# google-research/multinerf

Measured on NVIDIA H100. Metric: train-step rays/sec @16384 rays x (64+64+32) samples, higher is better.
Workload: dtype bf16

## Files before the change

### include/mnrf.h

```cpp
#ifndef MNRF_H_
#define MNRF_H_

#include <stddef.h>
#include <stdint.h>

#ifdef __cplusplus
extern "C" {
#endif

typedef uint16_t mnrf_bf16;
typedef void* mnrf_stream;

#define MNRF_ABI_VERSION 2

int mnrf_abi_version(void);
const char* mnrf_last_error(void);
int mnrf_device_ok(void);
int mnrf_num_sms(void);

typedef struct {
  int32_t num_rays, num_prev, num_samples;
  int32_t use_dilation;
  float dilation, domain_lo, domain_hi;
  float anneal, resample_padding;
// ... 33 lines not shown
                     mnrf_stream stream);

enum { MNRF_GEMM_FWD = 0, MNRF_GEMM_DGRAD = 1, MNRF_GEMM_WGRAD = 2 };
enum { MNRF_ACT_NONE = 0, MNRF_ACT_RELU = 1, MNRF_ACT_SOFTPLUS = 2, MNRF_ACT_SILU = 3 };

typedef struct {
  int32_t mode, act;
  int64_t m;
  int32_t n, k;
  int64_t lda, ldb, ldc, ldmask;
  int64_t ldmaskbits;
  int64_t ldadd;
  int64_t mask_mod;
  int32_t impl;
} mnrf_gemm_desc;

int mnrf_gemm(const mnrf_gemm_desc* d, const mnrf_bf16* a, const mnrf_bf16* b, const float* bias,
              const float* rowv, const float* colv, const mnrf_bf16* mask, uint32_t* maskbits,
              float* colsum, const mnrf_bf16* addend, mnrf_bf16* z, int64_t ldz, void* out, mnrf_stream stream);

int mnrf_gemm_wgrad(const mnrf_gemm_desc* d, const mnrf_bf16* a, const mnrf_bf16* b, float* bsum,
                    const float* side_w, float* side_aw, float* out, mnrf_stream stream);

typedef struct {
  int32_t block_n;
  int32_t staged;
  int32_t mask_tma;
  int32_t smooth;
  int32_t side;
  int32_t splits;
  int32_t tiles;
  int32_t grid;
  int32_t pingpong;
} mnrf_gemm_instance;
int mnrf_gemm_plan(const mnrf_gemm_desc* d, const mnrf_bf16* a, const mnrf_bf16* b, const float* bias,
                   const float* rowv, const float* colv, const mnrf_bf16* mask, const uint32_t* maskbits,
                   const float* colsum, const mnrf_bf16* addend, const mnrf_bf16* z, int64_t ldz, const void* out,
                   const float* bsum, const float* side_w, const float* side_aw, mnrf_gemm_instance* plan);

#define MNRF_CHAIN_MAX_LAYERS 8
enum { MNRF_CHAIN_FWD = 0, MNRF_CHAIN_BWD = 1 };

typedef struct {
  const mnrf_bf16* w;
  int64_t ldw;
  const float* bias;
  uint32_t* maskbits;
  int64_t ldmaskbits;
  float* colsum;
  mnrf_bf16* out;
  int64_t ldo;
  int32_t n_stream, stream_col0, stream_kb0;
  int32_t n_res, res_kb0;
  int32_t reserved;
} mnrf_chain_layer;

typedef struct {
  int32_t mode, num_layers;
  int32_t width;
  int32_t stream_cols;
  int64_t m;
  const mnrf_bf16* stream;
  int64_t ldstream;
  const float* head_w;
  const float* head_b;
  float* head_out;
// ... 200 lines not shown
```

### multinerf_b200/csrc/gemm_tc.cu

```cuda
#include <cuda.h>

#include <stdlib.h>
#include <string.h>

#include <algorithm>

#include "tc_common.cuh"

namespace mnrf {

constexpr int BLOCK_M = 128;
constexpr int BLOCK_K = 64;
constexpr int A_STAGE_BYTES = BLOCK_M * BLOCK_K * 2;
constexpr int NUM_THREADS = 384;
constexpr int CS_MAX = 1024;
constexpr int gemm_stages(int bn) { return bn == 256 ? 4 : bn == 128 ? 6 : 8; }
constexpr int STAGING_BLOCK_BYTES = 64 * 128;
constexpr int staging_blocks(int mode, int bn, bool ts) {
  return !ts ? 0 : (mode == MNRF_GEMM_FWD && bn >= 128) ? 2 : 1;
}
constexpr int mask_words(int bn) { return bn >= 128 ? bn / 32 : 0; }
constexpr int MASK_BUFS = 2;
constexpr int dgrad_smem_bytes(int bn) { return 8 * bn * 4 + MASK_BUFS * BLOCK_M * mask_words(bn) * 4; }
constexpr int SIDE_SCRATCH = 96 * 8;
// ... 75 lines not shown
          w = r < 32 ? wl : wh;
        }
        if (r < BLOCK_K) {
          const uint4 v = ld_shared_v4((base + r * 128) ^ ((r & 7) << 4));
          const uint32_t u[4] = {v.x, v.y, v.z, v.w};
#pragma unroll
          for (int q = 0; q < 4; ++q) {
            acc[2 * q] = fmaf(w, bf16_lo(u[q]), acc[2 * q]);
            acc[2 * q + 1] = fmaf(w, bf16_hi(u[q]), acc[2 * q + 1]);
          }
        }
      }
      __syncwarp();
      if (lane == 0) mbar_arrive(&empty_bar[slot % STAGES]);
    }
    if (own < BLOCK_K && kb0 < kb1) {
      if (NT > 32) named_bar_sync(4, NT); else __syncwarp();
#pragma unroll
      for (int e = 0; e < 8; ++e) st_shared_u32(scratch + (t * 8 + e) * 4, __float_as_uint(acc[e]));
      if (NT > 32) named_bar_sync(4, NT); else __syncwarp();
      const int64_t col0 = WEIGHTED ? (int64_t)m_blk * BLOCK_M : (int64_t)n_blk * COLS;
      float* out = WEIGHTED ? p.side_aw : p.bsum;
      for (int col = t; col < COLS; col += NT) {
        if (WEIGHTED && col0 + col >= p.m) break;
        float sum = 0.f;
#pragma unroll
        for (int g = 0; g < G; ++g) sum += __uint_as_float(ld_shared_u32(scratch + (g * COLS + col) * 4));
        atomicAdd(out + col0 + col, sum);
      }
    }
  }
}

template <int MODE, int NC, bool TS, int SB, bool SMOOTH>
__device__ __forceinline__ void gemm_epilogue(const GemmParams& p, const CUtensorMap* tmap_c, const float (&acc)[NC / 2],
                                              int m_blk, int r0, int ncol0, int wg, uint8_t* smem_c, bool mask_tma,
                                              uint32_t m_tile, bool do_cs, uint32_t cs_lane) {
  constexpr int MW = mask_words(NC);
  const int lane = threadIdx.x & 31;
  const int r_in = r0 + (16 * ((threadIdx.x >> 5) & 3) + (lane >> 2));
  const int cq = 2 * (lane & 3);
  const bool leader = (threadIdx.x & 127) == 0;
  const uint32_t c_row = smem_u32(smem_c) + wg * (SB * STAGING_BLOCK_BYTES) + (r_in - r0) * 128 + (cq << 1);
  const uint32_t m_row = m_tile + r_in * (MW * 4);
  int64_t rows[2];
  bool row_ok[2];
  float rv[2] = {0.f, 0.f};
  const uint32_t* mrow[2] = {nullptr, nullptr};
#pragma unroll
  for (int h = 0; h < 2; ++h) {
    rows[h] = (int64_t)m_blk * BLOCK_M + r_in + 8 * h;
    row_ok[h] = rows[h] < p.m;
    if (MODE == MNRF_GEMM_DGRAD && row_ok[h]) {
      if (p.rowv) rv[h] = p.rowv[rows[h]];
      if (p.maskbits && !mask_tma)
        mrow[h] = p.maskbits + (p.mask_mod > 0 ? rows[h] % p.mask_mod : rows[h]) * p.ldmaskbits;
    }
  }
  uint32_t bits[2] = {0u, 0u};
  uint32_t mw[2] = {0u, 0u};
#pragma unroll
  for (int i = 0; i < NC / 8; ++i) {
    const int col = ncol0 + 8 * i + cq;
    if (TS && SB == 1 && (i & 7) == 0) {
      if (leader) tma_store_wait_read<0>();
      named_bar_sync(2 + wg, 128);
    }
    if (MODE == MNRF_GEMM_DGRAD && p.maskbits && (i & 3) == 0) {
#pragma unroll
      for (int h = 0; h < 2; ++h)
        mw[h] = mask_tma ? ld_shared_u32(m_row + (8 * h * MW + (i >> 2)) * 4)
                         : row_ok[h] ? __ldg(mrow[h] + (col >> 5)) : 0u;
    }
    float v[2][2];
#pragma unroll
    for (int h = 0; h < 2; ++h) { v[h][0] = acc[4 * i + 2 * h]; v[h][1] = acc[4 * i + 2 * h + 1]; }
    if (MODE == MNRF_GEMM_FWD) {
      if (p.bias) {
        const float2 b = __ldg(reinterpret_cast<const float2*>(p.bias + col));
#pragma unroll
        for (int h = 0; h < 2; ++h) { v[h][0] += b.x; v[h][1] += b.y; }
      }
      if constexpr (SMOOTH) {
#pragma unroll
        for (int h = 0; h < 2; ++h) {
          if (p.mask && row_ok[h])
            *reinterpret_cast<uint32_t*>(const_cast<__nv_bfloat16*>(p.mask) + rows[h] * p.ldmask + col) =
                pack_bf16(v[h][0], v[h][1]);
          v[h][0] = act_fwd(p.act, v[h][0]);
          v[h][1] = act_fwd(p.act, v[h][1]);
        }
      } else if (p.act == MNRF_ACT_RELU) {
#pragma unroll
        for (int h = 0; h < 2; ++h)
#pragma unroll
          for (int e = 0; e < 2; ++e) {
            v[h][e] = relu_nan(v[h][e]);
            bits[h] |= (v[h][e] > 0.f ? 1u : 0u) << ((8 * i + cq + e) & 31);
          }
      }
    } else {
      float2 cv = make_float2(0.f, 0.f);
      if (p.rowv) cv = __ldg(reinterpret_cast<const float2*>(p.colv + col));
#pragma unroll
      for (int h = 0; h < 2; ++h) {
        if (p.rowv) { v[h][0] += rv[h] * cv.x; v[h][1] += rv[h] * cv.y; }
        if constexpr (SMOOTH) {
          if (row_ok[h]) {
            const int64_t zr = p.mask_mod > 0 ? rows[h] % p.mask_mod : rows[h];
            const uint32_t zz = __ldg(reinterpret_cast<const unsigned int*>(p.mask + zr * p.ldmask + col));
            v[h][0] *= act_d1(p.act, bf16_lo(zz));
            v[h][1] *= act_d1(p.act, bf16_hi(zz));
          }
        } else if (p.maskbits) {
          if (!((mw[h] >> (col & 31)) & 1u)) v[h][0] = 0.f;
          if (!((mw[h] >> ((col + 1) & 31)) & 1u)) v[h][1] = 0.f;
        } else if (p.mask && row_ok[h]) {
          const uint32_t mm = __ldg(reinterpret_cast<const unsigned int*>(p.mask + rows[h] * p.ldmask + col));
          if (!(bf16_lo(mm) > 0.f)) v[h][0] = 0.f;
          if (!(bf16_hi(mm) > 0.f)) v[h][1] = 0.f;
        }
        if (p.addend && row_ok[h]) {
          const uint32_t aa = __ldg(reinterpret_cast<const unsigned int*>(p.addend + rows[h] * p.ldadd + col));
          v[h][0] += bf16_lo(aa);
          v[h][1] += bf16_hi(aa);
        }
      }
      if (do_cs) {
        const bool hi = (lane >> 2) & 1;
        const float s0 = v[0][0] + v[1][0], s1 = v[0][1] + v[1][1];
        float t = (hi ? s1 : s0) + __shfl_xor_sync(0xffffffffu, hi ? s0 : s1, 4);
        t += __shfl_xor_sync(0xffffffffu, t, 8);
        t += __shfl_xor_sync(0xffffffffu, t, 16);
        if (lane < 8) {
          const uint32_t a = cs_lane + 8 * i * 4;
          st_shared_u32(a, __float_as_uint(__uint_as_float(ld_shared_u32(a)) + t));
        }
      }
    }
#pragma unroll
    for (int h = 0; h < 2; ++h) {
      if (TS) {
        st_shared_u32(c_row + ((i >> 3) & (SB - 1)) * STAGING_BLOCK_BYTES + h * (8 * 128) +
                          (((i & 7) ^ ((lane >> 2) & 7)) << 4),
                      pack_bf16(v[h][0], v[h][1]));
      } else if (row_ok[h]) {
        *reinterpret_cast<uint32_t*>(reinterpret_cast<__nv_bfloat16*>(p.out) + rows[h] * p.ldc + col) =
            pack_bf16(v[h][0], v[h][1]);
      }
    }
    if (MODE == MNRF_GEMM_FWD && p.act == MNRF_ACT_RELU && p.maskbits && (i & 3) == 3) {
#pragma unroll
      for (int h = 0; h < 2; ++h) {
        bits[h] |= __shfl_xor_sync(0xffffffffu, bits[h], 1);
        bits[h] |= __shfl_xor_sync(0xffffffffu, bits[h], 2);
        if ((lane & 3) == ((i >> 2) & 3) && row_ok[h]) p.maskbits[rows[h] * p.ldmaskbits + (col >> 5)] = bits[h];
        bits[h] = 0u;
      }
    }
    if (TS && (i & 7) == 7) {
      fence_proxy_async();
      if (SB == 2 && leader) tma_store_wait_read<0>();
      named_bar_sync(2 + wg, 128);
      if (leader) {
        tma_store_2d(tmap_c, smem_c + (wg * SB + ((i >> 3) & (SB - 1))) * STAGING_BLOCK_BYTES, ncol0 + 8 * (i & ~7),
                     (int)((int64_t)m_blk * BLOCK_M + r0));
        tma_store_commit();
      }
    }
  }
}

template <int MODE, int BN, bool TS, bool SIDE, bool SMOOTH = false>
__global__ void __launch_bounds__(NUM_THREADS, 1)
gemm_tc_kernel(const __grid_constant__ CUtensorMap tmap_a, const __grid_constant__ CUtensorMap tmap_b,
               const __grid_constant__ CUtensorMap tmap_c, const __grid_constant__ CUtensorMap tmap_m,
               const GemmParams p) {
  constexpr int STAGES = gemm_stages(BN);
  constexpr int B_STAGE = BN * BLOCK_K * 2;
  constexpr bool kWgrad = (MODE == MNRF_GEMM_WGRAD);
  constexpr bool kDgrad = (MODE == MNRF_GEMM_DGRAD);
  constexpr int NACC = BN / 2;
  constexpr int SB = staging_blocks(MODE, BN, TS);
  constexpr int MW = mask_words(BN);
  static_assert(SB < 2 || (BN / 64) % 2 == 0, "block j of every tile must use staging block j % SB");
  static_assert(!SIDE || kWgrad, "side sums are a WGRAD feature");
  static_assert(!SMOOTH || (TS && !kWgrad), "smooth activations are FWD / DGRAD epilogues of the staged store");
  extern __shared__ uint8_t smem_dyn[];
  uint8_t* smem = reinterpret_cast<uint8_t*>((reinterpret_cast<uintptr_t>(smem_dyn) + 1023) & ~uintptr_t(1023));
  uint8_t* smem_a = smem;
  uint8_t* smem_b = smem + STAGES * A_STAGE_BYTES;
  uint8_t* smem_c = smem_b + STAGES * B_STAGE;
  float* cs_s = reinterpret_cast<float*>(smem_c + 2 * SB * STAGING_BLOCK_BYTES);
  float* side_s = cs_s;
  uint32_t* mask_s = reinterpret_cast<uint32_t*>(cs_s + (kDgrad ? 8 * BN : SIDE ? SIDE_SCRATCH : 0));
  uint64_t* full_bar = reinterpret_cast<uint64_t*>(mask_s + (kDgrad ? MASK_BUFS * BLOCK_M * MW : 0));
  uint64_t* empty_bar = full_bar + STAGES;
  uint64_t* mask_full = empty_bar + STAGES;
  uint64_t* mask_empty = mask_full + MASK_BUFS;

  const int warp = threadIdx.x >> 5;
// ... 93 lines not shown
          uint64_t adesc, bdesc;
          if (!kWgrad) {
            adesc = make_smem_desc(sa + c * (64 * 128) + k * (WGMMA_K * 2), 0, 1024);
            bdesc = make_smem_desc(sb + k * (WGMMA_K * 2), 0, 1024);
          } else {
            adesc = make_smem_desc(sa + c * (BLOCK_K * 128) + k * (WGMMA_K * 128), BLOCK_K * 128, 1024);
            bdesc = make_smem_desc(sb + k * (WGMMA_K * 128), BLOCK_K * 128, 1024);
          }
          Wgmma<BN, kWgrad ? 1 : 0, kWgrad ? 1 : 0>::mma(acc, adesc, bdesc, (kb > kb0 || k > 0) ? 1u : 0u);
        }
        wgmma_commit();
        wgmma_wait<1>();
        if (prev >= 0 && lane == 0) mbar_arrive(&empty_bar[prev]);
        prev = (int)stage;
        if (++stage == STAGES) { stage = 0; phase ^= 1; }
      }
      wgmma_wait<0>();
      fence_acc(acc);
      if (prev >= 0 && lane == 0) mbar_arrive(&empty_bar[prev]);

      const int ncol0 = n_blk * BN;
      if (MODE == MNRF_GEMM_WGRAD) {
#pragma unroll
        for (int h = 0; h < 2; ++h) {
          const int64_t row = (int64_t)m_blk * BLOCK_M + r_in + 8 * h;
          if (row >= p.m) continue;
          float* dst = reinterpret_cast<float*>(p.out) + row * p.ldc + ncol0 + cq;
#pragma unroll
          for (int i = 0; i < BN / 8; ++i) atomicAdd(reinterpret_cast<float2*>(dst + 8 * i), make_float2(acc[4 * i + 2 * h], acc[4 * i + 2 * h + 1]));
        }
        continue;
      }
      if (mask_tma) mbar_wait(&mask_full[it % MASK_BUFS], (it / MASK_BUFS) & 1, 5);
      gemm_epilogue<MODE, BN, TS, SB, SMOOTH>(p, &tmap_c, acc, m_blk, 64 * c, ncol0, c, smem_c, mask_tma,
                                              smem_u32(mask_s) + (it % MASK_BUFS) * (BLOCK_M * MW * 4), do_cs, cs_lane);
      if (mask_tma) {
        __syncwarp();
        if (lane == 0) mbar_arrive(&mask_empty[it % MASK_BUFS]);
      }
      const int next = tile + (int)gridDim.x;
      if (do_cs && (next >= total_tiles || next % p.num_n_blocks != n_blk)) {
        named_bar_sync(1, 2 * 128);
        for (int j = threadIdx.x - 128; j < BN; j += 2 * 128) {
          float s = 0.f;
#pragma unroll
          for (int sw = 0; sw < 8; ++sw) {
            s += cs_s[sw * BN + j];
            cs_s[sw * BN + j] = 0.f;
          }
          atomicAdd(p.colsum + ncol0 + j, s);
        }
        named_bar_sync(1, 2 * 128);
      }
    }
    if (TS && (threadIdx.x & 127) == 0) tma_store_wait_all();
  }
}

constexpr int PP_BN = 128;
constexpr int PP_STAGES = 5;
constexpr int PP_SB = 2;
constexpr int PP_MASK_BUFS = 4;
constexpr int pp_smem_bytes(int mode) {
  return PP_STAGES * (A_STAGE_BYTES + PP_BN * BLOCK_K * 2) + 2 * PP_SB * STAGING_BLOCK_BYTES +
         (mode == MNRF_GEMM_DGRAD ? PP_MASK_BUFS * BLOCK_M * mask_words(PP_BN) * 4 : 0) + 256  +
         1024 ;
}

template <int MODE, int BN>
__global__ void __launch_bounds__(NUM_THREADS, 1)
gemm_tc_pingpong_kernel(const __grid_constant__ CUtensorMap tmap_a, const __grid_constant__ CUtensorMap tmap_b,
                        const __grid_constant__ CUtensorMap tmap_c, const __grid_constant__ CUtensorMap tmap_m,
                        const GemmParams p) {
  constexpr int STAGES = PP_STAGES;
  constexpr int B_STAGE = PP_BN * BLOCK_K * 2;
  constexpr int SUB = BN / PP_BN;
  constexpr int MW = mask_words(PP_BN);
  constexpr int SB = PP_SB;
  constexpr bool kDgrad = (MODE == MNRF_GEMM_DGRAD);
  static_assert(MODE != MNRF_GEMM_WGRAD && (BN == 128 || BN == 256), "FWD / DGRAD tiles of 128 or 256 columns");
  extern __shared__ uint8_t smem_dyn[];
  uint8_t* smem = reinterpret_cast<uint8_t*>((reinterpret_cast<uintptr_t>(smem_dyn) + 1023) & ~uintptr_t(1023));
  uint8_t* smem_a = smem;
  uint8_t* smem_b = smem + STAGES * A_STAGE_BYTES;
  uint8_t* smem_c = smem_b + STAGES * B_STAGE;
  uint32_t* mask_s = reinterpret_cast<uint32_t*>(smem_c + 2 * SB * STAGING_BLOCK_BYTES);
  uint64_t* full_bar = reinterpret_cast<uint64_t*>(mask_s + (kDgrad ? PP_MASK_BUFS * BLOCK_M * MW : 0));
  uint64_t* empty_bar = full_bar + STAGES;
  uint64_t* mask_full = empty_bar + STAGES;
  uint64_t* mask_empty = mask_full + PP_MASK_BUFS;
  uint64_t* mma_turn = mask_empty + PP_MASK_BUFS;

  const int lane = threadIdx.x & 31;
  const int wg = threadIdx.x >> 7;
  const int total_tiles = p.num_m_blocks * p.num_n_blocks;
  const int nk = p.num_k_blocks;
  const bool mask_tma = kDgrad && p.mask_tma;

  if (threadIdx.x == 0) {
    prefetch_tmap(&tmap_a);
    prefetch_tmap(&tmap_b);
    prefetch_tmap(&tmap_c);
    if (mask_tma) prefetch_tmap(&tmap_m);
    for (int i = 0; i < STAGES; ++i) {
      mbar_init(&full_bar[i], 1);
      mbar_init(&empty_bar[i], 4);
    }
    for (int i = 0; i < PP_MASK_BUFS; ++i) {
      mbar_init(&mask_full[i], 1);
      mbar_init(&mask_empty[i], 4);
    }
    for (int i = 0; i < 2; ++i) mbar_init(&mma_turn[i], 4);
    fence_barrier_init();
  }
  __syncthreads();
  pdl_launch_dependents();
  pdl_wait();

  if (wg == 0) {
    setmaxnreg_dec<40>();
    if (threadIdx.x == 0) {
      uint32_t stage = 0, phase = 0;
      int it = 0;
      for (int tile = blockIdx.x; tile < total_tiles; tile += gridDim.x) {
        const int n_blk = tile % p.num_n_blocks;
        const int m_blk = tile / p.num_n_blocks;
        for (int s = 0; s < SUB; ++s, ++it) {
          const int ncol0 = n_blk * BN + s * PP_BN;
          if (mask_tma) {
            const int mb = it % PP_MASK_BUFS;
            mbar_wait(&mask_empty[mb], ((it / PP_MASK_BUFS) & 1) ^ 1, 4);
            mbar_expect_tx(&mask_full[mb], BLOCK_M * MW * 4);
            const int64_t r0 = (int64_t)m_blk * BLOCK_M;
            tma_load_2d(mask_s + mb * (BLOCK_M * MW), &tmap_m, &mask_full[mb], ncol0 / 32,
                        (int)(p.mask_mod > 0 ? r0 % p.mask_mod : r0));
          }
          for (int kb = 0; kb < nk; ++kb) {
            mbar_wait(&empty_bar[stage], phase ^ 1, 1);
            mbar_expect_tx(&full_bar[stage], A_STAGE_BYTES + B_STAGE);
            tma_load_2d(smem_a + stage * A_STAGE_BYTES, &tmap_a, &full_bar[stage], kb * BLOCK_K, m_blk * BLOCK_M);
            tma_load_2d(smem_b + stage * B_STAGE, &tmap_b, &full_bar[stage], kb * BLOCK_K, ncol0);
            if (++stage == STAGES) { stage = 0; phase ^= 1; }
          }
        }
      }
    }
  } else {
    setmaxnreg_inc<232>();
    const int c = wg - 1;
    float acc[2][64];
    for (int it = c; ; it += 2) {
      const int tile = blockIdx.x + (it / SUB) * (int)gridDim.x;
      if (tile >= total_tiles) break;
      const int s = it % SUB;
      const int n_blk = tile % p.num_n_blocks;
      const int m_blk = tile / p.num_n_blocks;
      const int ncol0 = n_blk * BN + s * PP_BN;
      const uint32_t slot = (uint32_t)it * (uint32_t)nk;
      uint32_t stage = slot % STAGES, phase = (slot / STAGES) & 1;
      if (it > 0) mbar_wait(&mma_turn[c], ((it - 1) >> 1) & 1, 7);
      int prev = -1;
      fence_acc(acc[0]);
      fence_acc(acc[1]);
      for (int kb = 0; kb < nk; ++kb) {
        mbar_wait(&full_bar[stage], phase, 3);
        const uint32_t sa = smem_u32(smem_a + stage * A_STAGE_BYTES);
        const uint32_t sb = smem_u32(smem_b + stage * B_STAGE);
        wgmma_fence();
#pragma unroll
        for (int k = 0; k < BLOCK_K / WGMMA_K; ++k) {
          const uint64_t bdesc = make_smem_desc(sb + k * (WGMMA_K * 2), 0, 1024);
#pragma unroll
          for (int g = 0; g < 2; ++g)
            Wgmma<PP_BN, 0, 0>::mma(acc[g], make_smem_desc(sa + g * (64 * 128) + k * (WGMMA_K * 2), 0, 1024), bdesc,
                                    (kb > 0 || k > 0) ? 1u : 0u);
        }
        wgmma_commit();
        wgmma_wait<1>();
        if (prev >= 0 && lane == 0) mbar_arrive(&empty_bar[prev]);
        prev = (int)stage;
        if (++stage == STAGES) { stage = 0; phase ^= 1; }
      }
      if (blockIdx.x + ((it + 1) / SUB) * (int)gridDim.x < total_tiles) {
        __syncwarp();
        if (lane == 0) mbar_arrive(&mma_turn[c ^ 1]);
      }
      wgmma_wait<0>();
      fence_acc(acc[0]);
      fence_acc(acc[1]);
      if (prev >= 0 && lane == 0) mbar_arrive(&empty_bar[prev]);

      const uint32_t m_base = smem_u32(mask_s) + (it % PP_MASK_BUFS) * (BLOCK_M * MW * 4);
      if (mask_tma) mbar_wait(&mask_full[it % PP_MASK_BUFS], (it / PP_MASK_BUFS) & 1, 5);
#pragma unroll 1
      for (int g = 0; g < 2; ++g) {
        gemm_epilogue<MODE, PP_BN, true, SB, false>(p, &tmap_c, acc[0], m_blk, 64 * g, ncol0, c, smem_c, mask_tma, m_base,
                                                    false, 0);
#pragma unroll
        for (int e = 0; e < 64; ++e) acc[0][e] = acc[1][e];
      }
      if (mask_tma) {
        __syncwarp();
        if (lane == 0) mbar_arrive(&mask_empty[it % PP_MASK_BUFS]);
      }
    }
    if ((threadIdx.x & 127) == 0) tma_store_wait_all();
  }
}

template <int MODE, int BN>
static int launch_gemm_tc_pingpong(int grid, const CUtensorMap& ta, const CUtensorMap& tb, const CUtensorMap& tc,
                                   const CUtensorMap& tm, const GemmParams& p, cudaStream_t stream) {
  constexpr int kSmem = pp_smem_bytes(MODE);
  static_assert(kSmem <= 232448, "shared memory budget");
  return launch_tc<gemm_tc_pingpong_kernel<MODE, BN>>(grid, NUM_THREADS, kSmem, stream, ta, tb, tc, tm, p);
}

template <int MODE, int BN, bool TS, bool SIDE, bool SMOOTH = false>
static int launch_gemm_tc(int grid, const CUtensorMap& ta, const CUtensorMap& tb, const CUtensorMap& tc,
                          const CUtensorMap& tm, const GemmParams& p, cudaStream_t stream) {
  constexpr int kSmem = smem_bytes(MODE, BN, TS, SIDE);
  static_assert(kSmem <= 232448, "shared memory budget");
  return launch_tc<gemm_tc_kernel<MODE, BN, TS, SIDE, SMOOTH>>(grid, NUM_THREADS, kSmem, stream, ta, tb, tc, tm, p);
}

int gemm_tc_smooth_launch(int mode, int block_n, int grid, const CUtensorMap& ta, const CUtensorMap& tb,
                          const CUtensorMap& tc, const GemmParams& p, cudaStream_t stream);

#ifndef MNRF_GEMM_TC_SMOOTH_UNIT
static int pick_block_n(int n) {
  const int cands[] = {256, 128, 64, 32, 16};
  for (int c : cands)
    if (n % c == 0) return c;
  return 0;
}

static int gemm_tc_plan(const mnrf_gemm_desc* d, const mnrf_bf16* a, const mnrf_bf16* b, const float* bias,
                        const float* colv, const mnrf_bf16* mask, const uint32_t* maskbits, const float* colsum,
                        const mnrf_bf16* addend, const void* out, const float* bsum, const float* side_w,
                        const float* side_aw, const mnrf_bf16* z, int64_t ldz, mnrf_gemm_instance* plan,
                        GemmParams* p) {
  MNRF_CHECK(d->mode == MNRF_GEMM_WGRAD || d->k % BLOCK_K == 0,
             "mnrf_gemm(tc): reduction length %d must be a multiple of %d", d->k, BLOCK_K);
  MNRF_CHECK(d->lda % 8 == 0 && d->ldb % 8 == 0 && ((uintptr_t)a % 16) == 0 && ((uintptr_t)b % 16) == 0,
             "mnrf_gemm(tc): operands must be 16-byte aligned with ld %% 8 == 0");
  const int block_n = pick_block_n(d->n);
  MNRF_CHECK(block_n > 0, "mnrf_gemm(tc): N=%d must be a multiple of 16", d->n);
  if (d->mode == MNRF_GEMM_WGRAD)
// ... 18 lines not shown
  }
  if (bias) MNRF_CHECK(((uintptr_t)bias % 8) == 0, "mnrf_gemm(tc): bias must be 8-byte aligned");
  if (colv) MNRF_CHECK(((uintptr_t)colv % 8) == 0, "mnrf_gemm(tc): colv must be 8-byte aligned");
  const int workers = mnrf_num_sms();
  const int num_m_blocks = (int)((d->m + BLOCK_M - 1) / BLOCK_M);
  const int num_n_blocks = d->n / block_n;
  const int num_k_blocks = (d->k + BLOCK_K - 1) / BLOCK_K;
  int num_splits = 1;
  if (d->mode == MNRF_GEMM_WGRAD) {
    const int out_tiles = num_m_blocks * num_n_blocks;
    const int max_splits = std::min(std::max(1, (2 * workers) / out_tiles), num_k_blocks);
    int splits = max_splits;
    for (int sp = 1; sp <= max_splits; ++sp) {
      const int items = out_tiles * sp;
      const int rounds = (items + workers - 1) / workers;
      if (items * 100 >= rounds * workers * 95) { splits = sp; break; }
    }
    num_splits = splits;
  }
  const int kblocks_per_split = (num_k_blocks + num_splits - 1) / num_splits;
  num_splits = (num_k_blocks + kblocks_per_split - 1) / kblocks_per_split;
  if (d->mode != MNRF_GEMM_WGRAD) {
    MNRF_CHECK(d->ldc % 2 == 0 && ((uintptr_t)out % 4) == 0, "mnrf_gemm(tc): bf16 output must be 4-byte aligned");
    if (mask) MNRF_CHECK(d->ldmask % 2 == 0 && ((uintptr_t)mask % 4) == 0, "mnrf_gemm(tc): mask must be 4-byte aligned");
  } else {
    MNRF_CHECK(d->ldc % 2 == 0 && ((uintptr_t)out % 8) == 0, "mnrf_gemm(tc): fp32 output must be 8-byte aligned");
  }
  const bool ts = d->mode != MNRF_GEMM_WGRAD && block_n >= 64 && ((uintptr_t)out % 16) == 0 && d->ldc % 8 == 0;
  MNRF_CHECK(!smooth || ts, "mnrf_gemm(tc): a smooth activation needs N %% 64 == 0 and a 16-byte aligned output "
             "with a row pitch that is a multiple of 8");
  const bool mask_tma = d->mode == MNRF_GEMM_DGRAD && maskbits && mask_words(block_n) > 0 && d->ldmaskbits % 4 == 0 &&
                        ((uintptr_t)maskbits % 16) == 0 && (d->mask_mod == 0 || d->mask_mod % BLOCK_M == 0);
  const bool pingpong = d->mode != MNRF_GEMM_WGRAD && ts && d->n % PP_BN == 0 && !smooth && !colsum;
  const int tiles = num_m_blocks * num_n_blocks * num_splits;
  plan->block_n = block_n;
  plan->staged = ts;
  plan->mask_tma = mask_tma;
  plan->smooth = smooth;
  plan->side = side;
  plan->splits = num_splits;
  plan->tiles = tiles;
  plan->grid = std::min(tiles, workers);
  plan->pingpong = pingpong;
  p->num_m_blocks = num_m_blocks;
  p->num_n_blocks = num_n_blocks;
  p->num_k_blocks = num_k_blocks;
  p->num_splits = num_splits;
  p->kblocks_per_split = kblocks_per_split;
  return 0;
}

template <int MODE>
static int launch_register_store(int block_n, int grid, const CUtensorMap& ta, const CUtensorMap& tb,
                                 const CUtensorMap& tc, const CUtensorMap& tm, const GemmParams& p,
                                 cudaStream_t stream) {
  switch (block_n) {
    case 256: return launch_gemm_tc<MODE, 256, false, false>(grid, ta, tb, tc, tm, p, stream);
    case 128: return launch_gemm_tc<MODE, 128, false, false>(grid, ta, tb, tc, tm, p, stream);
    case 64: return launch_gemm_tc<MODE, 64, false, false>(grid, ta, tb, tc, tm, p, stream);
    case 32: return launch_gemm_tc<MODE, 32, false, false>(grid, ta, tb, tc, tm, p, stream);
    case 16: return launch_gemm_tc<MODE, 16, false, false>(grid, ta, tb, tc, tm, p, stream);
  }
  set_error("mnrf_gemm(tc): no register-store instance at BN=%d", block_n);
  return 1;
}

static int launch_gemm_tc_plan(int mode, const mnrf_gemm_instance& plan, const CUtensorMap& ta, const CUtensorMap& tb,
                               const CUtensorMap& tc, const CUtensorMap& tm, const GemmParams& p,
                               cudaStream_t stream) {
  const int bn = plan.block_n, grid = plan.grid;
  const bool fwd = mode == MNRF_GEMM_FWD;
  if (plan.pingpong) {
    if (bn == 256)
      return fwd ? launch_gemm_tc_pingpong<MNRF_GEMM_FWD, 256>(grid, ta, tb, tc, tm, p, stream)
                 : launch_gemm_tc_pingpong<MNRF_GEMM_DGRAD, 256>(grid, ta, tb, tc, tm, p, stream);
    if (bn == 128)
      return fwd ? launch_gemm_tc_pingpong<MNRF_GEMM_FWD, 128>(grid, ta, tb, tc, tm, p, stream)
                 : launch_gemm_tc_pingpong<MNRF_GEMM_DGRAD, 128>(grid, ta, tb, tc, tm, p, stream);
  } else if (plan.smooth) {
    return gemm_tc_smooth_launch(mode, bn, grid, ta, tb, tc, p, stream);
  } else if (mode == MNRF_GEMM_WGRAD) {
    if (bn == 256)
      return plan.side ? launch_gemm_tc<MNRF_GEMM_WGRAD, 256, false, true>(grid, ta, tb, tc, tm, p, stream)
                       : launch_gemm_tc<MNRF_GEMM_WGRAD, 256, false, false>(grid, ta, tb, tc, tm, p, stream);
    if (bn == 128)
      return plan.side ? launch_gemm_tc<MNRF_GEMM_WGRAD, 128, false, true>(grid, ta, tb, tc, tm, p, stream)
                       : launch_gemm_tc<MNRF_GEMM_WGRAD, 128, false, false>(grid, ta, tb, tc, tm, p, stream);
    if (bn == 64)
      return plan.side ? launch_gemm_tc<MNRF_GEMM_WGRAD, 64, false, true>(grid, ta, tb, tc, tm, p, stream)
                       : launch_gemm_tc<MNRF_GEMM_WGRAD, 64, false, false>(grid, ta, tb, tc, tm, p, stream);
  } else if (!plan.staged) {
    return fwd ? launch_register_store<MNRF_GEMM_FWD>(bn, grid, ta, tb, tc, tm, p, stream)
               : launch_register_store<MNRF_GEMM_DGRAD>(bn, grid, ta, tb, tc, tm, p, stream);
  } else if (bn == 64) {
    return fwd ? launch_gemm_tc<MNRF_GEMM_FWD, 64, true, false>(grid, ta, tb, tc, tm, p, stream)
               : launch_gemm_tc<MNRF_GEMM_DGRAD, 64, true, false>(grid, ta, tb, tc, tm, p, stream);
  } else if (!fwd) {
    if (bn == 256) return launch_gemm_tc<MNRF_GEMM_DGRAD, 256, true, false>(grid, ta, tb, tc, tm, p, stream);
    if (bn == 128) return launch_gemm_tc<MNRF_GEMM_DGRAD, 128, true, false>(grid, ta, tb, tc, tm, p, stream);
  }
  set_error("mnrf_gemm(tc): no kernel instance for mode %d, BN=%d, staged %d, side sums %d", mode, bn, plan.staged,
            plan.side);
  return 1;
}

int gemm_tc_launch(const mnrf_gemm_desc* d, const mnrf_bf16* a, const mnrf_bf16* b, const float* bias,
                   const float* rowv, const float* colv, const mnrf_bf16* mask, uint32_t* maskbits,
                   float* colsum, const mnrf_bf16* addend, void* out, cudaStream_t stream, float* bsum,
                   const float* side_w, float* side_aw, mnrf_bf16* z, int64_t ldz) {
  mnrf_gemm_instance plan;
  GemmParams p{};
// ... 30 lines not shown
  if (ts) {
    if (make_tmap(&tc, out, d->m, d->n, d->ldc, 64, 64)) return 1;
  } else {
    tc = tb;
  }
  CUtensorMap tm = tb;
  if (p.mask_tma &&
      make_tmap(&tm, maskbits, d->mask_mod > 0 ? d->mask_mod : d->m, d->n / 32, d->ldmaskbits,
                mask_words(plan.pingpong ? PP_BN : block_n), BLOCK_M, CU_TENSOR_MAP_DATA_TYPE_UINT32, 4,
                CU_TENSOR_MAP_SWIZZLE_NONE))
    return 1;
  if (plan.grid == 0) return 0;
  if (int rc = launch_gemm_tc_plan(d->mode, plan, ta, tb, tc, tm, p, stream)) return rc;
  MNRF_LAUNCH_CHECK();
  return 0;
}
#endif

}

#ifndef MNRF_GEMM_TC_SMOOTH_UNIT
extern "C" int mnrf_gemm_plan(const mnrf_gemm_desc* d, const mnrf_bf16* a, const mnrf_bf16* b, const float* bias,
                              const float* rowv, const float* colv, const mnrf_bf16* mask, const uint32_t* maskbits,
                              const float* colsum, const mnrf_bf16* addend, const mnrf_bf16* z, int64_t ldz,
                              const void* out, const float* bsum, const float* side_w, const float* side_aw,
                              mnrf_gemm_instance* plan) {
  MNRF_CHECK(d && plan, "mnrf_gemm_plan: null pointer");
  MNRF_CHECK((rowv == nullptr) == (colv == nullptr), "mnrf_gemm: rowv and colv come together");
  MNRF_CHECK(!mask || d->mask_mod == 0, "mnrf_gemm: mask_mod applies to maskbits and z, not to a bf16 mask");
  mnrf::GemmParams p;
  return mnrf::gemm_tc_plan(d, a, b, bias, colv, mask, maskbits, colsum, addend, out, bsum, side_w, side_aw, z, ldz,
                            plan, &p);
}
#endif
```

### multinerf_b200/lib.py

```python
import ctypes as C
import os

import torch

_HERE = os.path.dirname(os.path.abspath(__file__))
LIB_PATH = os.environ.get('MNRF_LIB') or os.path.join(_HERE, 'libmnrf_b200.so')


class MnrfError(RuntimeError):
  pass


class SampleDesc(C.Structure):
  _fields_ = [('num_rays', C.c_int32), ('num_prev', C.c_int32), ('num_samples', C.c_int32),
              ('use_dilation', C.c_int32), ('dilation', C.c_float), ('domain_lo', C.c_float),
              ('domain_hi', C.c_float), ('anneal', C.c_float), ('resample_padding', C.c_float),
              ('jitter_mode', C.c_int32), ('max_jitter', C.c_float)]


class EncodeDesc(C.Structure):
  _fields_ = [('num_rays', C.c_int32), ('num_samples', C.c_int32), ('raydist_fn', C.c_int32),
              ('ray_shape', C.c_int32), ('warp_contract', C.c_int32),
              ('disable_integration', C.c_int32), ('basis_k', C.c_int32), ('min_deg', C.c_int32),
              ('max_deg', C.c_int32), ('ld_feat', C.c_int32), ('feat_cols', C.c_int32)]


class GemmDesc(C.Structure):
  _fields_ = [('mode', C.c_int32), ('act', C.c_int32), ('m', C.c_int64), ('n', C.c_int32),
              ('k', C.c_int32), ('lda', C.c_int64), ('ldb', C.c_int64), ('ldc', C.c_int64),
              ('ldmask', C.c_int64), ('ldmaskbits', C.c_int64), ('ldadd', C.c_int64),
              ('mask_mod', C.c_int64),
              ('impl', C.c_int32)]


class GemmInstance(C.Structure):
  _fields_ = [('block_n', C.c_int32), ('staged', C.c_int32), ('mask_tma', C.c_int32), ('smooth', C.c_int32),
              ('side', C.c_int32), ('splits', C.c_int32), ('tiles', C.c_int32), ('grid', C.c_int32),
              ('pingpong', C.c_int32)]


class HeadInstance(C.Structure):
  _fields_ = [('fwd_kernel', C.c_int32), ('fwd_lpr', C.c_int32), ('fwd_grid', C.c_int32), ('bwd_kernel', C.c_int32),
              ('bwd_n_out', C.c_int32), ('bwd_lpr', C.c_int32), ('bwd_chunks', C.c_int32), ('bwd_smooth', C.c_int32),
              ('bwd_grid', C.c_int32), ('reserved', C.c_int32), ('fwd_rows_per_pass', C.c_int64),
              ('bwd_rows_per_block', C.c_int64)]


class CompositeDesc(C.Structure):
  _fields_ = [('num_rays', C.c_int32), ('num_samples', C.c_int32), ('raydist_fn', C.c_int32),
              ('opaque_background', C.c_int32), ('density_bias', C.c_float),
              ('density_noise', C.c_float), ('rgb_act', C.c_int32), ('rgb_premult', C.c_float),
              ('rgb_bias', C.c_float), ('rgb_padding', C.c_float), ('bg_const', C.c_float),
              ('rgb_mode', C.c_int32), ('ld_density', C.c_int32), ('ld_rgb', C.c_int32)]


class LossDesc(C.Structure):
  _fields_ = [('c', CompositeDesc), ('loss_type', C.c_int32), ('charb_padding', C.c_float),
              ('data_mult', C.c_float), ('distortion_mult', C.c_float),
              ('interlevel_mult', C.c_float), ('num_samples_fine', C.c_int32),
              ('lossmult_channels', C.c_int32)]


class RobustDesc(C.Structure):
  _fields_ = [('num_rays', C.c_int32), ('patch_size', C.c_int32), ('inner_patch_size', C.c_int32),
              ('filter_size', C.c_int32), ('enable', C.c_int32), ('smoothed_thresh', C.c_float),
              ('patch_thresh', C.c_float)]


class RefdirDesc(C.Structure):
  _fields_ = [('M', C.c_int64), ('num_samples', C.c_int32), ('use_pred_normals', C.c_int32),
              ('use_density_normals', C.c_int32), ('use_reflections', C.c_int32), ('use_ide', C.c_int32),
# ... 153 lines not shown
```

Before: 275,400.

## Specialize pingpong DGRAD epilogue operands and triple-buffer its TMA store staging

Adds compile-time epilogue variants for the pingpong DGRAD GEMM when the operands are fixed to TMA-loaded mask bits, with or without the rank-1 rowv/colv term, so runtime null-pointer branches drop out. The pingpong DGRAD kernel also moves to three staging blocks per warpgroup. The staging block index now rotates across calls, and the code waits only until one TMA store is outstanding instead of draining all of them. This is meant to cut store-wait stalls in the epilogue, at the cost of more shared memory and extra template instantiations. Optional clock64 instrumentation is added behind a compile flag.

```diff
diff --git a/include/mnrf.h b/include/mnrf.h
--- a/include/mnrf.h
+++ b/include/mnrf.h
@@ -89,6 +89,7 @@
   int32_t tiles;
   int32_t grid;
   int32_t pingpong;
+  int32_t epilogue;
 } mnrf_gemm_instance;
 int mnrf_gemm_plan(const mnrf_gemm_desc* d, const mnrf_bf16* a, const mnrf_bf16* b, const float* bias,
                    const float* rowv, const float* colv, const mnrf_bf16* mask, const uint32_t* maskbits,
diff --git a/multinerf_b200/csrc/gemm_tc.cu b/multinerf_b200/csrc/gemm_tc.cu
--- a/multinerf_b200/csrc/gemm_tc.cu
+++ b/multinerf_b200/csrc/gemm_tc.cu
@@ -131,11 +131,41 @@
   }
 }
 
-template <int MODE, int NC, bool TS, int SB, bool SMOOTH>
+enum { GK_TURN, GK_FULL, GK_MMA, GK_EPI_LOOP, GK_EPI_SYNC, GK_MASK, GK_N };
+#ifdef MNRF_GEMM_CLOCKS
+__device__ unsigned long long g_gemm_clk[2][GK_N];
+struct GemmClk {
+  long long t[GK_N] = {};
+  long long last = 0;
+  __device__ __forceinline__ void start() { last = clock64(); }
+  __device__ __forceinline__ void tick(int k) {
+    const long long now = clock64();
+    t[k] += now - last;
+    last = now;
+  }
+};
+#else
+struct GemmClk {
+  __device__ __forceinline__ void start() {}
+  __device__ __forceinline__ void tick(int) {}
+};
+#endif
+
+enum { EPI_GENERIC = 0, EPI_BITS_TMA = 1, EPI_BITS_TMA_RANK1 = 2 };
+
+template <int MODE, int NC, bool TS, int SB, bool SMOOTH, int OPS = EPI_GENERIC>
 __device__ __forceinline__ void gemm_epilogue(const GemmParams& p, const CUtensorMap* tmap_c, const float (&acc)[NC / 2],
                                               int m_blk, int r0, int ncol0, int wg, uint8_t* smem_c, bool mask_tma,
-                                              uint32_t m_tile, bool do_cs, uint32_t cs_lane) {
+                                              uint32_t m_tile, bool do_cs, uint32_t cs_lane, int& sblk, GemmClk& clk) {
   constexpr int MW = mask_words(NC);
+  static_assert(OPS == EPI_GENERIC || (MODE == MNRF_GEMM_DGRAD && TS && !SMOOTH && MW > 0),
+                "fixed operand sets are DGRAD epilogues of the staged store with TMA-loaded mask bits");
+  constexpr bool kFixed = OPS != EPI_GENERIC;
+  const bool has_rowv = kFixed ? OPS == EPI_BITS_TMA_RANK1 : p.rowv != nullptr;
+  const bool has_bits = kFixed || p.maskbits != nullptr;
+  const bool bits_tma = kFixed || mask_tma;
+  const bool has_mask = !kFixed && p.mask != nullptr;
+  const bool has_addend = !kFixed && p.addend != nullptr;
   const int lane = threadIdx.x & 31;
   const int r_in = r0 + (16 * ((threadIdx.x >> 5) & 3) + (lane >> 2));
   const int cq = 2 * (lane & 3);
@@ -151,8 +181,8 @@
     rows[h] = (int64_t)m_blk * BLOCK_M + r_in + 8 * h;
     row_ok[h] = rows[h] < p.m;
     if (MODE == MNRF_GEMM_DGRAD && row_ok[h]) {
-      if (p.rowv) rv[h] = p.rowv[rows[h]];
-      if (p.maskbits && !mask_tma)
+      if (has_rowv) rv[h] = p.rowv[rows[h]];
+      if (has_bits && !bits_tma)
         mrow[h] = p.maskbits + (p.mask_mod > 0 ? rows[h] % p.mask_mod : rows[h]) * p.ldmaskbits;
     }
   }
@@ -161,14 +191,17 @@
 #pragma unroll
   for (int i = 0; i < NC / 8; ++i) {
     const int col = ncol0 + 8 * i + cq;
+    const int sb = SB == 3 ? sblk : (i >> 3) & (SB - 1);
     if (TS && SB == 1 && (i & 7) == 0) {
+      clk.tick(GK_EPI_LOOP);
       if (leader) tma_store_wait_read<0>();
       named_bar_sync(2 + wg, 128);
-    }
-    if (MODE == MNRF_GEMM_DGRAD && p.maskbits && (i & 3) == 0) {
+      clk.tick(GK_EPI_SYNC);
+    }
+    if (MODE == MNRF_GEMM_DGRAD && has_bits && (i & 3) == 0) {
 #pragma unroll
       for (int h = 0; h < 2; ++h)
-        mw[h] = mask_tma ? ld_shared_u32(m_row + (8 * h * MW + (i >> 2)) * 4)
+        mw[h] = bits_tma ? ld_shared_u32(m_row + (8 * h * MW + (i >> 2)) * 4)
                          : row_ok[h] ? __ldg(mrow[h] + (col >> 5)) : 0u;
     }
     float v[2][2];
@@ -200,10 +233,10 @@
       }
     } else {
       float2 cv = make_float2(0.f, 0.f);
-      if (p.rowv) cv = __ldg(reinterpret_cast<const float2*>(p.colv + col));
+      if (has_rowv) cv = __ldg(reinterpret_cast<const float2*>(p.colv + col));
 #pragma unroll
       for (int h = 0; h < 2; ++h) {
-        if (p.rowv) { v[h][0] += rv[h] * cv.x; v[h][1] += rv[h] * cv.y; }
+        if (has_rowv) { v[h][0] += rv[h] * cv.x; v[h][1] += rv[h] * cv.y; }
         if constexpr (SMOOTH) {
           if (row_ok[h]) {
             const int64_t zr = p.mask_mod > 0 ? rows[h] % p.mask_mod : rows[h];
@@ -211,15 +244,15 @@
             v[h][0] *= act_d1(p.act, bf16_lo(zz));
             v[h][1] *= act_d1(p.act, bf16_hi(zz));
           }
-        } else if (p.maskbits) {
+        } else if (has_bits) {
           if (!((mw[h] >> (col & 31)) & 1u)) v[h][0] = 0.f;
           if (!((mw[h] >> ((col + 1) & 31)) & 1u)) v[h][1] = 0.f;
-        } else if (p.mask && row_ok[h]) {
+        } else if (has_mask && row_ok[h]) {
           const uint32_t mm = __ldg(reinterpret_cast<const unsigned int*>(p.mask + rows[h] * p.ldmask + col));
           if (!(bf16_lo(mm) > 0.f)) v[h][0] = 0.f;
           if (!(bf16_hi(mm) > 0.f)) v[h][1] = 0.f;
         }
-        if (p.addend && row_ok[h]) {
+        if (has_addend && row_ok[h]) {
           const uint32_t aa = __ldg(reinterpret_cast<const unsigned int*>(p.addend + rows[h] * p.ldadd + col));
           v[h][0] += bf16_lo(aa);
           v[h][1] += bf16_hi(aa);
@@ -240,8 +273,7 @@
 #pragma unroll
     for (int h = 0; h < 2; ++h) {
       if (TS) {
-        st_shared_u32(c_row + ((i >> 3) & (SB - 1)) * STAGING_BLOCK_BYTES + h * (8 * 128) +
-                          (((i & 7) ^ ((lane >> 2) & 7)) << 4),
+        st_shared_u32(c_row + sb * STAGING_BLOCK_BYTES + h * (8 * 128) + (((i & 7) ^ ((lane >> 2) & 7)) << 4),
                       pack_bf16(v[h][0], v[h][1]));
       } else if (row_ok[h]) {
         *reinterpret_cast<uint32_t*>(reinterpret_cast<__nv_bfloat16*>(p.out) + rows[h] * p.ldc + col) =
@@ -259,13 +291,16 @@
     }
     if (TS && (i & 7) == 7) {
       fence_proxy_async();
-      if (SB == 2 && leader) tma_store_wait_read<0>();
+      clk.tick(GK_EPI_LOOP);
+      if (SB >= 2 && leader) tma_store_wait_read<SB - 2>();
       named_bar_sync(2 + wg, 128);
       if (leader) {
-        tma_store_2d(tmap_c, smem_c + (wg * SB + ((i >> 3) & (SB - 1))) * STAGING_BLOCK_BYTES, ncol0 + 8 * (i & ~7),
+        tma_store_2d(tmap_c, smem_c + (wg * SB + sb) * STAGING_BLOCK_BYTES, ncol0 + 8 * (i & ~7),
                      (int)((int64_t)m_blk * BLOCK_M + r0));
         tma_store_commit();
       }
+      if (SB == 3) sblk = sblk == 2 ? 0 : sblk + 1;
+      clk.tick(GK_EPI_SYNC);
     }
   }
 }
@@ -425,8 +460,12 @@
         continue;
       }
       if (mask_tma) mbar_wait(&mask_full[it % MASK_BUFS], (it / MASK_BUFS) & 1, 5);
+      int sblk = 0;
+      GemmClk clk;
+      clk.start();
       gemm_epilogue<MODE, BN, TS, SB, SMOOTH>(p, &tmap_c, acc, m_blk, 64 * c, ncol0, c, smem_c, mask_tma,
-                                              smem_u32(mask_s) + (it % MASK_BUFS) * (BLOCK_M * MW * 4), do_cs, cs_lane);
+                                              smem_u32(mask_s) + (it % MASK_BUFS) * (BLOCK_M * MW * 4), do_cs, cs_lane,
+                                              sblk, clk);
       if (mask_tma) {
         __syncwarp();
         if (lane == 0) mbar_arrive(&mask_empty[it % MASK_BUFS]);
@@ -452,15 +491,15 @@
 
 constexpr int PP_BN = 128;
 constexpr int PP_STAGES = 5;
-constexpr int PP_SB = 2;
+constexpr int pp_staging_blocks(int mode) { return mode == MNRF_GEMM_DGRAD ? 3 : 2; }
 constexpr int PP_MASK_BUFS = 4;
 constexpr int pp_smem_bytes(int mode) {
-  return PP_STAGES * (A_STAGE_BYTES + PP_BN * BLOCK_K * 2) + 2 * PP_SB * STAGING_BLOCK_BYTES +
+  return PP_STAGES * (A_STAGE_BYTES + PP_BN * BLOCK_K * 2) + 2 * pp_staging_blocks(mode) * STAGING_BLOCK_BYTES +
          (mode == MNRF_GEMM_DGRAD ? PP_MASK_BUFS * BLOCK_M * mask_words(PP_BN) * 4 : 0) + 256  +
          1024 ;
 }
 
-template <int MODE, int BN>
+template <int MODE, int BN, int OPS>
 __global__ void __launch_bounds__(NUM_THREADS, 1)
 gemm_tc_pingpong_kernel(const __grid_constant__ CUtensorMap tmap_a, const __grid_constant__ CUtensorMap tmap_b,
                         const __grid_constant__ CUtensorMap tmap_c, const __grid_constant__ CUtensorMap tmap_m,
@@ -469,7 +508,7 @@
   constexpr int B_STAGE = PP_BN * BLOCK_K * 2;
   constexpr int SUB = BN / PP_BN;
   constexpr int MW = mask_words(PP_BN);
-  constexpr int SB = PP_SB;
+  constexpr int SB = pp_staging_blocks(MODE);
   constexpr bool kDgrad = (MODE == MNRF_GEMM_DGRAD);
   static_assert(MODE != MNRF_GEMM_WGRAD && (BN == 128 || BN == 256), "FWD / DGRAD tiles of 128 or 256 columns");
   extern __shared__ uint8_t smem_dyn[];
@@ -488,7 +527,7 @@
   const int wg = threadIdx.x >> 7;
   const int total_tiles = p.num_m_blocks * p.num_n_blocks;
   const int nk = p.num_k_blocks;
-  const bool mask_tma = kDgrad && p.mask_tma;
+  const bool mask_tma = kDgrad && (OPS != EPI_GENERIC || p.mask_tma);
 
   if (threadIdx.x == 0) {
     prefetch_tmap(&tmap_a);
@@ -542,6 +581,9 @@
     setmaxnreg_inc<232>();
     const int c = wg - 1;
     float acc[2][64];
+    int sblk = 0;
+    GemmClk clk;
+    clk.start();
     for (int it = c; ; it += 2) {
       const int tile = blockIdx.x + (it / SUB) * (int)gridDim.x;
       if (tile >= total_tiles) break;
@@ -551,12 +593,15 @@
       const int ncol0 = n_blk * BN + s * PP_BN;
       const uint32_t slot = (uint32_t)it * (uint32_t)nk;
       uint32_t stage = slot % STAGES, phase = (slot / STAGES) & 1;
+      clk.tick(GK_EPI_LOOP);
       if (it > 0) mbar_wait(&mma_turn[c], ((it - 1) >> 1) & 1, 7);
+      clk.tick(GK_TURN);
       int prev = -1;
       fence_acc(acc[0]);
       fence_acc(acc[1]);
       for (int kb = 0; kb < nk; ++kb) {
         mbar_wait(&full_bar[stage], phase, 3);
+        clk.tick(GK_FULL);
         const uint32_t sa = smem_u32(smem_a + stage * A_STAGE_BYTES);
         const uint32_t sb = smem_u32(smem_b + stage * B_STAGE);
         wgmma_fence();
@@ -573,6 +618,7 @@
         if (prev >= 0 && lane == 0) mbar_arrive(&empty_bar[prev]);
         prev = (int)stage;
         if (++stage == STAGES) { stage = 0; phase ^= 1; }
+        clk.tick(GK_MMA);
       }
       if (blockIdx.x + ((it + 1) / SUB) * (int)gridDim.x < total_tiles) {
         __syncwarp();
@@ -582,13 +628,15 @@
       fence_acc(acc[0]);
       fence_acc(acc[1]);
       if (prev >= 0 && lane == 0) mbar_arrive(&empty_bar[prev]);
+      clk.tick(GK_MMA);
 
       const uint32_t m_base = smem_u32(mask_s) + (it % PP_MASK_BUFS) * (BLOCK_M * MW * 4);
       if (mask_tma) mbar_wait(&mask_full[it % PP_MASK_BUFS], (it / PP_MASK_BUFS) & 1, 5);
+      clk.tick(GK_MASK);
 #pragma unroll 1
       for (int g = 0; g < 2; ++g) {
-        gemm_epilogue<MODE, PP_BN, true, SB, false>(p, &tmap_c, acc[0], m_blk, 64 * g, ncol0, c, smem_c, mask_tma, m_base,
-                                                    false, 0);
+        gemm_epilogue<MODE, PP_BN, true, SB, false, OPS>(p, &tmap_c, acc[0], m_blk, 64 * g, ncol0, c, smem_c, mask_tma,
+                                                         m_base, false, 0, sblk, clk);
 #pragma unroll
         for (int e = 0; e < 64; ++e) acc[0][e] = acc[1][e];
       }
@@ -598,15 +646,32 @@
       }
     }
     if ((threadIdx.x & 127) == 0) tma_store_wait_all();
-  }
-}
-
-template <int MODE, int BN>
+#ifdef MNRF_GEMM_CLOCKS
+    clk.tick(GK_EPI_SYNC);
+    if (blockIdx.x == 0 && (threadIdx.x & 127) == 0)
+      for (int k = 0; k < GK_N; ++k) atomicAdd(&g_gemm_clk[c][k], (unsigned long long)clk.t[k]);
+#endif
+  }
+}
+
+template <int MODE, int BN, int OPS = EPI_GENERIC>
 static int launch_gemm_tc_pingpong(int grid, const CUtensorMap& ta, const CUtensorMap& tb, const CUtensorMap& tc,
                                    const CUtensorMap& tm, const GemmParams& p, cudaStream_t stream) {
   constexpr int kSmem = pp_smem_bytes(MODE);
   static_assert(kSmem <= 232448, "shared memory budget");
-  return launch_tc<gemm_tc_pingpong_kernel<MODE, BN>>(grid, NUM_THREADS, kSmem, stream, ta, tb, tc, tm, p);
+  return launch_tc<gemm_tc_pingpong_kernel<MODE, BN, OPS>>(grid, NUM_THREADS, kSmem, stream, ta, tb, tc, tm, p);
+}
+
+template <int BN>
+static int launch_dgrad_pingpong(int ops, int grid, const CUtensorMap& ta, const CUtensorMap& tb, const CUtensorMap& tc,
+                                 const CUtensorMap& tm, const GemmParams& p, cudaStream_t stream) {
+  switch (ops) {
+    case EPI_BITS_TMA:
+      return launch_gemm_tc_pingpong<MNRF_GEMM_DGRAD, BN, EPI_BITS_TMA>(grid, ta, tb, tc, tm, p, stream);
+    case EPI_BITS_TMA_RANK1:
+      return launch_gemm_tc_pingpong<MNRF_GEMM_DGRAD, BN, EPI_BITS_TMA_RANK1>(grid, ta, tb, tc, tm, p, stream);
+  }
+  return launch_gemm_tc_pingpong<MNRF_GEMM_DGRAD, BN>(grid, ta, tb, tc, tm, p, stream);
 }
 
 template <int MODE, int BN, bool TS, bool SIDE, bool SMOOTH = false>
@@ -691,6 +756,9 @@
   const bool mask_tma = d->mode == MNRF_GEMM_DGRAD && maskbits && mask_words(block_n) > 0 && d->ldmaskbits % 4 == 0 &&
                         ((uintptr_t)maskbits % 16) == 0 && (d->mask_mod == 0 || d->mask_mod % BLOCK_M == 0);
   const bool pingpong = d->mode != MNRF_GEMM_WGRAD && ts && d->n % PP_BN == 0 && !smooth && !colsum;
+  int epilogue = EPI_GENERIC;
+  if (pingpong && d->mode == MNRF_GEMM_DGRAD && mask_tma && !mask && !addend)
+    epilogue = colv ? EPI_BITS_TMA_RANK1 : EPI_BITS_TMA;
   const int tiles = num_m_blocks * num_n_blocks * num_splits;
   plan->block_n = block_n;
   plan->staged = ts;
@@ -701,6 +769,7 @@
   plan->tiles = tiles;
   plan->grid = std::min(tiles, workers);
   plan->pingpong = pingpong;
+  plan->epilogue = epilogue;
   p->num_m_blocks = num_m_blocks;
   p->num_n_blocks = num_n_blocks;
   p->num_k_blocks = num_k_blocks;
@@ -732,10 +801,10 @@
   if (plan.pingpong) {
     if (bn == 256)
       return fwd ? launch_gemm_tc_pingpong<MNRF_GEMM_FWD, 256>(grid, ta, tb, tc, tm, p, stream)
-                 : launch_gemm_tc_pingpong<MNRF_GEMM_DGRAD, 256>(grid, ta, tb, tc, tm, p, stream);
+                 : launch_dgrad_pingpong<256>(plan.epilogue, grid, ta, tb, tc, tm, p, stream);
     if (bn == 128)
       return fwd ? launch_gemm_tc_pingpong<MNRF_GEMM_FWD, 128>(grid, ta, tb, tc, tm, p, stream)
-                 : launch_gemm_tc_pingpong<MNRF_GEMM_DGRAD, 128>(grid, ta, tb, tc, tm, p, stream);
+                 : launch_dgrad_pingpong<128>(plan.epilogue, grid, ta, tb, tc, tm, p, stream);
   } else if (plan.smooth) {
     return gemm_tc_smooth_launch(mode, bn, grid, ta, tb, tc, p, stream);
   } else if (mode == MNRF_GEMM_WGRAD) {
@@ -832,4 +901,13 @@
   return mnrf::gemm_tc_plan(d, a, b, bias, colv, mask, maskbits, colsum, addend, out, bsum, side_w, side_aw, z, ldz,
                             plan, &p);
 }
+
+#ifdef MNRF_GEMM_CLOCKS
+extern "C" int mnrf_gemm_clocks(unsigned long long* out) {
+  unsigned long long zero[2 * mnrf::GK_N] = {};
+  if (cudaDeviceSynchronize() != cudaSuccess) return 1;
+  if (cudaMemcpyFromSymbol(out, mnrf::g_gemm_clk, sizeof(zero)) != cudaSuccess) return 1;
+  return cudaMemcpyToSymbol(mnrf::g_gemm_clk, zero, sizeof(zero)) != cudaSuccess;
+}
 #endif
+#endif
diff --git a/multinerf_b200/lib.py b/multinerf_b200/lib.py
--- a/multinerf_b200/lib.py
+++ b/multinerf_b200/lib.py
@@ -36,7 +36,7 @@
 class GemmInstance(C.Structure):
   _fields_ = [('block_n', C.c_int32), ('staged', C.c_int32), ('mask_tma', C.c_int32), ('smooth', C.c_int32),
               ('side', C.c_int32), ('splits', C.c_int32), ('tiles', C.c_int32), ('grid', C.c_int32),
-              ('pingpong', C.c_int32)]
+              ('pingpong', C.c_int32), ('epilogue', C.c_int32)]
 
 
 class HeadInstance(C.Structure):
```

Result: faster. 291,600 (median of 6 runs) (+5.9%).
